# XiangFeng-Wen/STF-Unet

Hardware: AMD Instinct MI355X
Metric: training samples/sec (256x256 DCE-MRI frames) (higher is better)
Workload: dtype bf16; 1 GPU; cfg2 UNet(in=8,base_c=64) 256x256 train step; model=UNet, global_batch=64, per_gpu_batch=64, seq_len=8, parallelism=dp1, ddp_hook=False

## Files before the change

include/stfunet.h:

```cpp
#ifndef STFUNET_H
#define STFUNET_H
#include <stddef.h>
#include <stdint.h>

#ifdef __cplusplus
extern "C" {
#endif

typedef void* stf_stream_t;

typedef struct stf_conv_geom {
  int N;
  int Hs, Ws, Cs;
  int src_cstride;
  int Hd, Wd;
  int R, S;
  int stride, pad;
  int transposed;
} stf_conv_geom;

typedef struct stf_lstm_epi {
  const float* c_prev;
  float* c_out;
  void* h_out;
// ... 78 lines not shown
               int res_cstride, const float* res_scale, const float* res_shift, void* out,
               int out_cstride, void* pooled, stf_stream_t stream);
int stf_bn_bwd_tiles(int N, int H, int W, int C, int groups, int pooled);
int stf_bn_bwd_reduce(const void* dz, int dz_cstride, const void* dpool, const void* y,
                      int y_cstride, int N, int H, int W, int C, int groups,
                      const float* scale, const float* shift, const float* mean,
                      const float* invstd, int mask_mode, const void* mask_src,
                      int mask_cstride, void* g_out, float* partial, stf_stream_t stream);
int stf_bn_bwd_finalize(float* partial, int tiles, int groups, int C, int64_t M,
                        const float* gamma, const float* mean, const float* invstd,
                        float* dgamma, float* dbeta, float* coef, stf_stream_t stream);
typedef struct stf_bn_gsum_desc {
  const float* partial;
  float* dgamma;
  float* dbeta;
  int tiles, groups, C;
} stf_bn_gsum_desc;
int stf_bn_groupsum_batch(const stf_bn_gsum_desc* descs, int count, stf_stream_t stream);
int stf_bn_bwd_apply_tiles(int64_t M, int C);
int stf_bn_bwd_apply(const void* g, int g_cstride, const void* y, int y_cstride, int64_t M,
                     int C, int groups, const float* mask_scale, const float* mask_shift,
                     const float* coef, void* dy, int dy_cstride, float* bias_partial,
                     float* dbias, stf_stream_t stream);

int stf_head_fwd(const void* y, int N, int H, int W, int C, const float* scale,
                 const float* shift, const float* w, const float* bias, int classes,
                 float* logits, stf_stream_t stream);
int stf_head_bwd(const float* dlogits, const void* y, int N, int H, int W, int C,
                 const float* scale, const float* shift, const float* mean,
                 const float* invstd, const float* w, int classes, void* g_out,
                 float* bn_partial, float* head_partial, float* dw, float* db,
                 stf_stream_t stream);
int stf_head_tiles(int N, int H, int W, int C);

int stf_loss_scratch_floats(int N, int classes);
int stf_loss_fwd(const float* logits, const int64_t* target, int N, int H, int W,
                 int classes, float* terms, float* loss, stf_stream_t stream);
int stf_loss_bwd(const float* logits, const int64_t* target, int N, int H, int W,
                 int classes, const float* terms, const float* grad_out, float* dlogits,
                 stf_stream_t stream);
int stf_loss_opt_scratch_floats(int N, int classes);
int stf_loss_opt_fwd(const float* logits, const int64_t* target, int N, int H, int W, int classes,
                     const float* class_weight, int ignore_index, int dice, float* terms,
                     float* loss, stf_stream_t stream);
int stf_loss_opt_bwd(const float* logits, const int64_t* target, int N, int H, int W, int classes,
                     const float* class_weight, int ignore_index, int dice, const float* terms,
                     const float* grad_out, float* dlogits, stf_stream_t stream);
int stf_head_mc_fwd(const void* y, int N, int H, int W, int C, const float* scale,
                    const float* shift, const float* w, const float* bias, int classes,
                    float* logits, stf_stream_t stream);
int stf_head_mc_bwd(const float* dlogits, const void* y, int N, int H, int W, int C,
                    const float* scale, const float* shift, const float* mean,
                    const float* invstd, const float* w, int classes, void* g_out,
                    float* bn_partial, float* head_partial, float* dw, float* db,
                    stf_stream_t stream);
int stf_loss_mc_scratch_floats(int N, int classes);
int stf_loss_mc_fwd(const float* logits, const int64_t* target, int N, int H, int W, int classes,
                    const float* class_weight, int ignore_index, int dice, float* terms,
                    float* loss, stf_stream_t stream);
int stf_loss_mc_bwd(const float* logits, const int64_t* target, int N, int H, int W, int classes,
                    const float* class_weight, int ignore_index, int dice, const float* terms,
                    const float* grad_out, float* dlogits, stf_stream_t stream);
int stf_loss_ft_scratch_floats(int N, int classes);
int stf_loss_ft_fwd(const float* logits, const int64_t* target, int N, int H, int W, int classes,
                    const float* class_weight, int ignore_index, int dice, float focal_gamma,
                    float tversky_alpha, float tversky_beta, float* terms, float* loss,
// ... 185 lines not shown
```

stf-unet_amd/csrc/bn.hip:

```cpp
#include <algorithm>

#include "common.h"
#include "../../include/stfunet.h"
#include "reduce.h"

namespace {

constexpr int NT = 256;

STF_DEV void bn_fin_store(int g, int c, int C, double mu, double var, const float* gamma, const float* beta,
                          float eps, float* mean, float* invstd, float* scale, float* shift) {
  const float inv = (float)(1.0 / sqrt(var + (double)eps));
  const float sc = gamma[c] * inv;
  mean[g * C + c] = (float)mu;
  invstd[g * C + c] = inv;
  scale[g * C + c] = sc;
  shift[g * C + c] = beta[c] - (float)mu * sc;
}

STF_DEV void bn_fin_fwd_out(float* base, int g, int c, int G, int C, long Mg, double s1, double s2,
                            const float* gamma, const float* beta, float mom, float eps, float* rm, float* rv,
                            float* mean, float* invstd, float* scale, float* shift) {
  const double mu = s1 / Mg;
  double var = s2 / Mg - mu * mu;
  if (var < 0) var = 0;
  bn_fin_store(g, c, C, mu, var, gamma, beta, eps, mean, invstd, scale, shift);
  if (G == 1) {
    if (!rm) return;
    const double unb = Mg > 1 ? var * Mg / (Mg - 1) : var;
    rm[c] = (1.f - mom) * rm[c] + mom * (float)mu;
    rv[c] = (1.f - mom) * rv[c] + mom * (float)unb;
  } else {
    base[c] = (float)mu;
    base[C + c] = (float)var;
  }
}

// ... 11 lines not shown
    stf::fold16_pair(base, S, 2L * C, C, c, cok, red, s1, s2);
    if (lead)
      bn_fin_fwd_out(base, g, c, G, C, Mg, s1, s2, gamma, beta, mom, eps, rm, rv, mean, invstd, scale, shift);
    return;
  }
  if (!lead) return;
  bn_fin_store(g, c, C, rm ? rm[c] : 0.f, rv ? rv[c] : 1.f, gamma, beta, eps, mean, invstd, scale, shift);
}

STF_DEV void bn_fin_bwd_out(float* base, int g, int c, int G, int C, long Mg, double s1, double s2,
                            const float* gamma, const float* mean, const float* invstd, float* dgamma, float* dbeta,
                            float* coef) {
  const double is = invstd[g * C + c];
  const double A = (double)gamma[c] * is;
  const double B = -A * is * s2 / Mg;
  const double Cc = -A * s1 / Mg + A * is * mean[g * C + c] * s2 / Mg;
  coef[(size_t)g * 3 * C + c] = (float)A;
  coef[(size_t)g * 3 * C + C + c] = (float)B;
  coef[(size_t)g * 3 * C + 2 * C + c] = (float)Cc;
  if (G == 1) {
    if (dgamma) dgamma[c] = (float)s2;
    if (dbeta) dbeta[c] = (float)s1;
  } else {
    base[c] = (float)s1;
    base[C + c] = (float)s2;
  }
}


STF_DEV void load_pair(const float* a, const float* b, int g, int C, int cg, float (&va)[8], float (&vb)[8]) {
  load8f(a + (size_t)g * C, cg * 8, va);
  load8f(b + (size_t)g * C, cg * 8, vb);
}
STF_DEV void load_coef(const float* coef, int g, int C, int cg, float (&A)[8], float (&B)[8], float (&Cc)[8]) {
  load8f(coef + (size_t)g * 3 * C, cg * 8, A);
  load8f(coef + (size_t)g * 3 * C + C, cg * 8, B);
  load8f(coef + (size_t)g * 3 * C + 2 * C, cg * 8, Cc);
}

STF_DEV void bn_affine8(float (&v)[8], const float (&sc)[8], const float (&sh)[8], int relu, int res_mode,
                        const uint4* rq, const float (&rs)[8], const float (&rh)[8]) {
#pragma unroll
  for (int j = 0; j < 8; ++j) v[j] = v[j] * sc[j] + sh[j];
  if (res_mode) {
    float r[8];
    unpack8(*rq, r);
    if (res_mode == 2) {
#pragma unroll
      for (int j = 0; j < 8; ++j) r[j] = r[j] * rs[j] + rh[j];
    }
#pragma unroll
    for (int j = 0; j < 8; ++j) v[j] += r[j];
  }
  if (relu) {
#pragma unroll
    for (int j = 0; j < 8; ++j) v[j] = fmaxf(v[j], 0.f);
  }
}

STF_DEV void bn_acc8(int mask, float (&d)[8], const float (&y)[8], const float (&sc)[8], const float (&sh)[8],
                     const float* mk, const float (&mu)[8], const float (&is)[8], float (&sg)[8], float (&sgx)[8]) {
#pragma unroll
  for (int j = 0; j < 8; ++j) {
    bool keep = true;
    if (mask == 1) keep = y[j] * sc[j] + sh[j] > 0.f;
    else if (mask == 2) keep = mk[j] > 0.f;
    const float gj = keep ? d[j] : 0.f;
    d[j] = gj;
    sg[j] += gj;
    sgx[j] += gj * (y[j] - mu[j]) * is[j];
  }
}

STF_DEV void bn_dy8(bool mask, float (&gv)[8], const float (&y)[8], const float (&ms)[8], const float (&mh)[8],
                    const float (&A)[8], const float (&B)[8], const float (&Cc)[8], float (&sb)[8]) {
#pragma unroll
  for (int j = 0; j < 8; ++j) {
    const float gj = (mask && !(y[j] * ms[j] + mh[j] > 0.f)) ? 0.f : gv[j];
    gv[j] = A[j] * gj + B[j] * y[j] + Cc[j];
    sb[j] += gv[j];
  }
}

template <int Q = 1, int NTH, int RW>
STF_DEV void bn_block_fold(float (&red)[NTH][RW], const float (&s0)[8], const float (&s1)[8], int C, int stride,
                           int gy, float* __restrict__ out) {
  constexpr int H = (RW - 1) / 8;
#pragma unroll
  for (int j = 0; j < 8; ++j) {
    red[threadIdx.x][j] = s0[j];
    if (H == 2) red[threadIdx.x][8 + j] = s1[j];
  }
  __syncthreads();
  const size_t row = (size_t)gy * gridDim.x + blockIdx.x;
  for (int c = threadIdx.x; c < C; c += NTH) {
    const int gg = c >> 3, j = c & 7;
    float a = 0.f, b = 0.f;
    for (int t = Q * gg; t < NTH; t += stride)
      for (int q = 0; q < Q; ++q) {
        a += red[t + q][j];
        if (H == 2) b += red[t + q][8 + j];
      }
    out[row * H * C + c] = a;
    if (H == 2) out[row * H * C + C + c] = b;
  }
}

template <bool POOL>
__global__ void bn_act_kernel(const uint16_t* __restrict__ y, int ycs, long N, int H, int W, int C, long Mg,
                              const float* scale, const float* shift, int relu, int res_mode,
                              const uint16_t* __restrict__ res, int rcs, const float* __restrict__ rscale,
                              const float* __restrict__ rshift, uint16_t* __restrict__ out, int ocs,
                              uint16_t* __restrict__ pooled) {
// ... 841 lines not shown
```

stf-unet_amd/csrc/head.hip:

```cpp
#include "common.h"
#include "../../include/stfunet.h"
#include "reduce.h"

namespace {

constexpr int NT = 256;

STF_DEV float lane_group_sum(float v, int CG) {
  if (CG >= 2) v += dpp_f<0xB1>(v);
  if (CG >= 4) v += dpp_f<0x4E>(v);
  if (CG >= 8) v += dpp_f<0x141>(v);
  if (CG >= 16) v += dpp_f<0x140>(v);
  for (int o = 16; o < CG; o <<= 1) v += __shfl_xor(v, o, 64);
  return v;
}

int head_tiles(long units) {
  long t = (units + NT - 1) / NT;
  return (int)(t < 1 ? 1 : (t > 1024 ? 1024 : t));
}

template <int K>
__global__ void head_fwd_kernel(const uint16_t* __restrict__ y, long P, int HW, int C,
                                const float* __restrict__ scale, const float* __restrict__ shift,
                                const float* __restrict__ w, const float* __restrict__ bias,
                                float* __restrict__ logits) {
  constexpr int U = 4;
  const int CG = C / 8, cgs = __builtin_ctz(CG);
  const int units = (int)(P * CG);
  const int cg = (int)((blockIdx.x * NT + threadIdx.x) & (CG - 1));
  float sc[8], sh[8], wk[K][8], bk[K];
  load8f(scale, cg * 8, sc);
  load8f(shift, cg * 8, sh);
#pragma unroll
  for (int k = 0; k < K; ++k) { load8f(w + k * C, cg * 8, wk[k]); bk[k] = bias[k]; }
  const int stride = gridDim.x * NT;
  for (int u0 = blockIdx.x * NT; u0 < units; u0 += stride * U) {
    uint4 raw[U];
#pragma unroll
    for (int r = 0; r < U; ++r) {
      const int u = u0 + r * stride + threadIdx.x;
      raw[r] = u < units ? *reinterpret_cast<const uint4*>(y + (size_t)(u >> cgs) * C + cg * 8) : make_uint4(0, 0, 0, 0);
    }
#pragma unroll
    for (int r = 0; r < U; ++r) {
      const int u = u0 + r * stride + threadIdx.x;
      float v[8], acc[K];
      unpack8(raw[r], v);
#pragma unroll
      for (int k = 0; k < K; ++k) acc[k] = 0.f;
#pragma unroll
      for (int j = 0; j < 8; ++j) {
        const float a = fmaxf(v[j] * sc[j] + sh[j], 0.f);
#pragma unroll
        for (int k = 0; k < K; ++k) acc[k] += a * wk[k][j];
      }
#pragma unroll
      for (int k = 0; k < K; ++k) acc[k] = lane_group_sum(acc[k], CG);
      if (u < units && cg == 0) {
        const int pix = u >> cgs, n = pix / HW, hw = pix - n * HW;
#pragma unroll
        for (int k = 0; k < K; ++k) logits[(size_t)(n * K + k) * HW + hw] = acc[k] + bk[k];
      }
    }
  }
}

template <int K>
__global__ void head_bwd_kernel(const float* __restrict__ dlogits, const uint16_t* __restrict__ y, long P, int HW,
                                int C, const float* __restrict__ scale, const float* __restrict__ shift,
                                const float* __restrict__ mean, const float* __restrict__ invstd,
                                const float* __restrict__ w, uint16_t* __restrict__ g_out,
                                float* __restrict__ bn_partial, float* __restrict__ head_partial) {
  constexpr int NV = 16 + 8 * K + K;
  __shared__ float red[NT][NV + 1];
  const int CG = C / 8, cgs = __builtin_ctz(CG);
  const int units = (int)(P * CG);
  const int gt = blockIdx.x * NT + threadIdx.x;
  const int cg = gt & (CG - 1);
  float sc[8], sh[8], mu[8], is[8], wk[K][8];
  load8f(scale, cg * 8, sc);
  load8f(shift, cg * 8, sh);
  load8f(mean, cg * 8, mu);
  load8f(invstd, cg * 8, is);
#pragma unroll
  for (int k = 0; k < K; ++k) load8f(w + k * C, cg * 8, wk[k]);
  float sg[8] = {0, 0, 0, 0, 0, 0, 0, 0}, sgx[8] = {0, 0, 0, 0, 0, 0, 0, 0}, dw[K][8], db[K];
#pragma unroll
  for (int k = 0; k < K; ++k) {
    db[k] = 0.f;
#pragma unroll
    for (int j = 0; j < 8; ++j) dw[k][j] = 0.f;
  }
  constexpr int U = 1;
  const int S = gridDim.x * NT;
  for (int u0 = gt; u0 < units; u0 += S * U) {
    float dlr[U][K];
    uint4 yr[U];
    int pixr[U];
#pragma unroll
    for (int r = 0; r < U; ++r) {
      const int u = u0 + r * S;
      const bool ok = u < units;
      const int pix = ok ? u >> cgs : 0, n = pix / HW, hw = pix - n * HW;
      pixr[r] = ok ? pix : -1;
#pragma unroll
      for (int k = 0; k < K; ++k) dlr[r][k] = ok ? dlogits[(size_t)(n * K + k) * HW + hw] : 0.f;
      yr[r] = ok ? *reinterpret_cast<const uint4*>(y + (size_t)pix * C + cg * 8) : make_uint4(0, 0, 0, 0);
    }
#pragma unroll
    for (int r = 0; r < U; ++r) {
    if (pixr[r] < 0) continue;
    const int pix = pixr[r];
    const float* dl = dlr[r];
    float v[8], g[8];
    unpack8(yr[r], v);
#pragma unroll
    for (int j = 0; j < 8; ++j) {
      const float z = v[j] * sc[j] + sh[j];
      const float a = fmaxf(z, 0.f);
      float da = 0.f;
#pragma unroll
      for (int k = 0; k < K; ++k) { da += dl[k] * wk[k][j]; dw[k][j] += dl[k] * a; }
      g[j] = z > 0.f ? da : 0.f;
      sg[j] += g[j];
      sgx[j] += g[j] * (v[j] - mu[j]) * is[j];
    }
    if (cg == 0) {
#pragma unroll
      for (int k = 0; k < K; ++k) db[k] += dl[k];
    }
    *reinterpret_cast<uint4*>(g_out + (size_t)pix * C + cg * 8) = pack8(g);
    }
  }
#pragma unroll
  for (int j = 0; j < 8; ++j) { red[threadIdx.x][j] = sg[j]; red[threadIdx.x][8 + j] = sgx[j]; }
#pragma unroll
  for (int k = 0; k < K; ++k) {
#pragma unroll
    for (int j = 0; j < 8; ++j) red[threadIdx.x][16 + k * 8 + j] = dw[k][j];
    red[threadIdx.x][16 + 8 * K + k] = db[k];
  }
  __syncthreads();
  for (int c = threadIdx.x; c < C; c += NT) {
    const int gg = c / 8, j = c - gg * 8;
    float a = 0.f, b = 0.f;
    for (int t = gg; t < NT; t += CG) { a += red[t][j]; b += red[t][8 + j]; }
    bn_partial[(size_t)blockIdx.x * 2 * C + c] = a;
    bn_partial[(size_t)blockIdx.x * 2 * C + C + c] = b;
  }
  const int HC = K * (C + 1);
  for (int e = threadIdx.x; e < HC; e += NT) {
    float a = 0.f;
    if (e < K * C) {
      const int k = e / C, c = e - k * C, gg = c / 8, j = c - gg * 8;
      for (int t = gg; t < NT; t += CG) a += red[t][16 + k * 8 + j];
    } else {
      const int k = e - K * C;
      for (int t = 0; t < NT; t += CG) a += red[t][16 + 8 * K + k];
    }
    head_partial[(size_t)blockIdx.x * HC + e] = a;
  }
}

__global__ void sum_tiles_kernel(const float* __restrict__ partial, int tiles, int C, int split,
// ... 84 lines not shown
                                                         float* __restrict__ bn_partial,
                                                         float* __restrict__ head_partial) {
  extern __shared__ __attribute__((aligned(16))) float sm[];
  const int CG = C / 8, cgs = __builtin_ctz(CG);
  const int units = (int)(P * CG);
  const int gt = blockIdx.x * NT + threadIdx.x;
  const int cg = gt & (CG - 1);
  const int K4 = (K + 3) & ~3;
  for (int i = threadIdx.x; i < K4 * C; i += NT) sm[i] = i < K * C ? w[i] : 0.f;
  float sc[8], sh[8], mu[8], is[8];
  load8f(scale, cg * 8, sc);
  load8f(shift, cg * 8, sh);
  load8f(mean, cg * 8, mu);
  load8f(invstd, cg * 8, is);
  float sg[8] = {0, 0, 0, 0, 0, 0, 0, 0}, sgx[8] = {0, 0, 0, 0, 0, 0, 0, 0}, dw[KP][8], db[KP];
#pragma unroll
  for (int k = 0; k < KP; ++k) {
    db[k] = 0.f;
#pragma unroll
    for (int j = 0; j < 8; ++j) dw[k][j] = 0.f;
  }
  __syncthreads();
  const float* wc = sm + cg * 8;
  const int S = gridDim.x * NT;
  for (int u = gt; u < units; u += S) {
    const int pix = u >> cgs, n = pix / HW, hw = pix - n * HW;
    const float* dp = dlogits + (size_t)n * K * HW + hw;
    float dl[KP];
#pragma unroll
    for (int k = 0; k < KP; ++k) dl[k] = k < K ? dp[(size_t)k * HW] : 0.f;
    const uint4 yr = *reinterpret_cast<const uint4*>(y + (size_t)pix * C + cg * 8);
    float v[8], a[8], g[8];
    unpack8(yr, v);
#pragma unroll
    for (int j = 0; j < 8; ++j) {
      a[j] = v[j] * sc[j] + sh[j];
      g[j] = 0.f;
    }
#pragma unroll
    for (int kb = 0; kb < KP; kb += 4) {
      if (kb < K) {
#pragma unroll
        for (int k = kb; k < kb + 4; ++k) {
          float wk[8];
          load8f(wc, k * C, wk);
#pragma unroll
          for (int j = 0; j < 8; ++j) {
            g[j] += dl[k] * wk[j];
            dw[k][j] += dl[k] * fmaxf(a[j], 0.f);
          }
        }
      }
    }
#pragma unroll
    for (int j = 0; j < 8; ++j) {
      g[j] = a[j] > 0.f ? g[j] : 0.f;
      sg[j] += g[j];
      sgx[j] += g[j] * (v[j] - mu[j]) * is[j];
    }
    if (cg == 0) {
#pragma unroll
      for (int k = 0; k < KP; ++k) db[k] += dl[k];
    }
    *reinterpret_cast<uint4*>(g_out + (size_t)pix * C + cg * 8) = pack8(g);
  }
  float(*red)[MCRED] = reinterpret_cast<float(*)[MCRED]>(sm);
  const int HC = K * (C + 1);
  __syncthreads();
#pragma unroll
  for (int j = 0; j < 8; ++j) { red[threadIdx.x][j] = sg[j]; red[threadIdx.x][8 + j] = sgx[j]; }
#pragma unroll
  for (int k = 0; k < KP; ++k) red[threadIdx.x][16 + k] = db[k];
  __syncthreads();
  for (int c = threadIdx.x; c < C; c += NT) {
    const int gg = c / 8, j = c - gg * 8;
    float a = 0.f, b = 0.f;
    for (int t = gg; t < NT; t += CG) { a += red[t][j]; b += red[t][8 + j]; }
    bn_partial[(size_t)blockIdx.x * 2 * C + c] = a;
    bn_partial[(size_t)blockIdx.x * 2 * C + C + c] = b;
  }
  if ((int)threadIdx.x < K) {
    float a = 0.f;
    for (int t = 0; t < NT; t += CG) a += red[t][16 + threadIdx.x];
    head_partial[(size_t)blockIdx.x * HC + K * C + threadIdx.x] = a;
  }
#pragma unroll
  for (int kb = 0; kb < KP; kb += 4) {
    if (kb < K) {
      __syncthreads();
#pragma unroll
      for (int kk = 0; kk < 4; ++kk)
#pragma unroll
        for (int j = 0; j < 8; ++j) red[threadIdx.x][kk * 8 + j] = dw[kb + kk][j];
      __syncthreads();
      for (int e = threadIdx.x; e < 4 * C; e += NT) {
        const int kk = e / C, c = e - kk * C, gg = c / 8, j = c - gg * 8;
        if (kb + kk < K) {
          float a = 0.f;
          for (int t = gg; t < NT; t += CG) a += red[t][kk * 8 + j];
          head_partial[(size_t)blockIdx.x * HC + (size_t)(kb + kk) * C + c] = a;
        }
      }
    }
  }
}

bool mc_classes_ok(int classes) { return classes >= 1 && classes <= MCK; }

constexpr long MCBLOCKS = 4096;
bool head_mc_units_ok(long HW, long units) { return HW < (1L << 31) && units < (1L << 31) - 2 * MCBLOCKS * NT; }

size_t head_mc_lds_bytes(int C, int classes, bool bwd) {
  size_t f = (size_t)((classes + 3) & ~3) * C;
  if (bwd && f < (size_t)NT * MCRED) f = (size_t)NT * MCRED;
  return f * sizeof(float);
}

}

extern "C" int stf_head_tiles(int N, int H, int W, int C) { return head_tiles((long)N * H * W * (C / 8)); }

extern "C" int stf_head_fwd(const void* y, int N, int H, int W, int C, const float* scale, const float* shift,
                            const float* w, const float* bias, int classes, float* logits, stf_stream_t stream) {
  if (!head_ok(C)) return STF_EINVAL;
  const long P = (long)N * H * W, units = P * (C / 8);
  if (units >= (1L << 31)) return STF_EINVAL;
  long blocks = (units + NT - 1) / NT;
  if (blocks > 8192) blocks = 8192;
  hipStream_t s = (hipStream_t)stream;
  STF_KDISPATCH(classes, hipLaunchKernelGGL(head_fwd_kernel<KK>, dim3(blocks), dim3(NT), 0, s, (const uint16_t*)y,
                                            P, H * W, C, scale, shift, w, bias, logits));
  STF_CHECK_LAUNCH();
  return 0;
}

// ... 8 lines not shown
  STF_KDISPATCH(classes, hipLaunchKernelGGL(head_bwd_kernel<KK>, dim3(tiles), dim3(NT), 0, s, dlogits,
                                            (const uint16_t*)y, P, H * W, C, scale, shift, mean, invstd, w,
                                            (uint16_t*)g_out, bn_partial, head_partial));
  STF_CHECK_LAUNCH();
  const int HC = classes * (C + 1);
  const int S = stf::colsum_stage1(head_partial, tiles, HC, s);
  hipLaunchKernelGGL(sum_tiles_kernel, dim3((HC + 255) / 256), dim3(256), 0, s, head_partial, S, HC, classes * C,
                     dw, db);
  STF_CHECK_LAUNCH();
  return 0;
}

extern "C" int stf_head_mc_fwd(const void* y, int N, int H, int W, int C, const float* scale, const float* shift,
                               const float* w, const float* bias, int classes, float* logits, stf_stream_t stream) {
  if (C < 8 || !head_ok(C) || !mc_classes_ok(classes) || N < 1 || H < 1 || W < 1) return STF_EINVAL;
  if (!y || !scale || !shift || !w || !bias || !logits) return STF_EINVAL;
  const long P = (long)N * H * W, units = P * (C / 8);
  if (!head_mc_units_ok((long)H * W, units)) return STF_EINVAL;
  long blocks = (units + NT - 1) / NT;
  if (blocks > MCBLOCKS) blocks = MCBLOCKS;
  hipStream_t s = (hipStream_t)stream;
  STF_KPDISPATCH(classes, hipLaunchKernelGGL(head_mc_fwd_kernel<KP>, dim3(blocks), dim3(NT),
                                             head_mc_lds_bytes(C, classes, false), s, (const uint16_t*)y, P, H * W, C,
                                             classes, scale, shift, w, bias, logits));
  STF_CHECK_LAUNCH();
  return 0;
}

extern "C" int stf_head_mc_bwd(const float* dlogits, const void* y, int N, int H, int W, int C, const float* scale,
                               const float* shift, const float* mean, const float* invstd, const float* w,
                               int classes, void* g_out, float* bn_partial, float* head_partial, float* dw, float* db,
                               stf_stream_t stream) {
  if (C < 8 || !head_ok(C) || !mc_classes_ok(classes) || N < 1 || H < 1 || W < 1) return STF_EINVAL;
  if (!dlogits || !y || !scale || !shift || !mean || !invstd || !w || !g_out || !bn_partial || !head_partial || !dw ||
      !db)
    return STF_EINVAL;
  if (!head_mc_units_ok((long)H * W, (long)N * H * W * (C / 8))) return STF_EINVAL;
  const long P = (long)N * H * W;
  const int tiles = stf_head_tiles(N, H, W, C);
  hipStream_t s = (hipStream_t)stream;
  STF_KPDISPATCH(classes, hipLaunchKernelGGL(head_mc_bwd_kernel<KP>, dim3(tiles), dim3(NT),
                                             head_mc_lds_bytes(C, classes, true), s, dlogits, (const uint16_t*)y, P,
                                             H * W, C, classes, scale, shift, mean, invstd, w, (uint16_t*)g_out,
                                             bn_partial, head_partial));
  STF_CHECK_LAUNCH();
  const int HC = classes * (C + 1);
  const int S = stf::colsum_stage1(head_partial, tiles, HC, s);
  hipLaunchKernelGGL(sum_tiles_kernel, dim3((HC + 255) / 256), dim3(256), 0, s, head_partial, S, HC, classes * C,
                     dw, db);
  STF_CHECK_LAUNCH();
  return 0;
}
```

stf-unet_amd/stfunet/_lib.py:

```python
import contextlib
import ctypes
import os

import torch

_HERE = os.path.dirname(os.path.abspath(__file__))
LIB_PATH = os.path.join(_HERE, "libstfunet_hip.so")
LIB_PATH = os.environ.get("STF_LIB", LIB_PATH)
LIB_PATH_F16 = os.environ.get("STF_LIB_F16", os.path.join(os.path.dirname(LIB_PATH), "libstfunet_hip_f16.so"))
LIB_PATHS = {torch.bfloat16: LIB_PATH, torch.float16: LIB_PATH_F16}
STORAGE_CODE = {torch.bfloat16: 0, torch.float16: 1}

BUILD_INFO = os.path.join(_HERE, "build_info.json")
_SRC_DIRS = (os.path.join(_HERE, "..", "csrc"), os.path.join(_HERE, "..", "..", "include"))


def _sha(paths):
    import hashlib
    h = hashlib.sha256()
    for p in paths:
        h.update(os.path.basename(p).encode())
        with open(p, "rb") as f:
            h.update(f.read())
    return h.hexdigest()[:16]
# ... 59 lines not shown
    _fields_ = [("g", ConvGeom), ("dy", P), ("dy_cstride", c_int), ("Nout", c_int), ("x", P),
                ("ws", P), ("splits", c_int), ("grid_blocks", c_int)]


class Seg(ctypes.Structure):
    _fields_ = [("off", c_int64), ("len", c_int64)]


_SIGS = {
    "stf_igemm_stat_tiles": (c_int, [ctypes.POINTER(IgemmArgs)]),
    "stf_igemm_ws_bytes": (c_size_t, [ctypes.POINTER(IgemmArgs)]),
    "stf_igemm_bnr_tiles": (c_int, [ctypes.POINTER(IgemmArgs)]),
    "stf_igemm_kernel_name": (ctypes.c_char_p, [ctypes.POINTER(IgemmArgs)]),
    "stf_wgrad_kernel_name": (ctypes.c_char_p, [ctypes.POINTER(WgradArgs)]),
    "stf_igemm": (c_int, [ctypes.POINTER(IgemmArgs), P]),
    "stf_wgrad_plan": (c_int, [ctypes.POINTER(WgradArgs), ctypes.POINTER(c_int), ctypes.POINTER(c_size_t)]),
    "stf_wgrad": (c_int, [ctypes.POINTER(WgradArgs), P]),
    "stf_wgrad_reduce": (c_int, [P, c_int, c_int, c_int, c_int, c_int, P, P]),
    "stf_channel_sum": (c_int, [P, c_int, c_int, c_int, P, P, P]),
    "stf_bn_finalize": (c_int, [P, c_int, c_int, c_int, c_int64, P, P, c_float, c_float, P, P, P, P, P, P, P]),
    "stf_bn_running_batch": (c_int, [P, c_int, P]),
    "stf_bn_groupsum_batch": (c_int, [P, c_int, P]),
    "stf_bn_act": (c_int, [P, c_int, c_int, c_int, c_int, c_int, c_int, P, P, c_int, P, c_int, P, P, P, c_int, P,
                           P]),
    "stf_bn_bwd_tiles": (c_int, [c_int, c_int, c_int, c_int, c_int, c_int]),
    "stf_bn_bwd_reduce": (c_int, [P, c_int, P, P, c_int, c_int, c_int, c_int, c_int, c_int, P, P, P, P, c_int, P,
                                  c_int, P, P, P]),
    "stf_bn_bwd_finalize": (c_int, [P, c_int, c_int, c_int, c_int64, P, P, P, P, P, P, P]),
    "stf_bn_bwd_apply_tiles": (c_int, [c_int64, c_int]),
    "stf_bn_bwd_apply": (c_int, [P, c_int, P, c_int, c_int64, c_int, c_int, P, P, P, P, c_int, P, P, P]),
    "stf_head_fwd": (c_int, [P, c_int, c_int, c_int, c_int, P, P, P, P, c_int, P, P]),
    "stf_head_bwd": (c_int, [P, P, c_int, c_int, c_int, c_int, P, P, P, P, P, c_int, P, P, P, P, P, P]),
    "stf_head_tiles": (c_int, [c_int, c_int, c_int, c_int]),
    "stf_loss_scratch_floats": (c_int, [c_int, c_int]),
    "stf_loss_fwd": (c_int, [P, P, c_int, c_int, c_int, c_int, P, P, P]),
    "stf_loss_bwd": (c_int, [P, P, c_int, c_int, c_int, c_int, P, P, P, P]),
    "stf_loss_opt_scratch_floats": (c_int, [c_int, c_int]),
    "stf_loss_opt_fwd": (c_int, [P, P, c_int, c_int, c_int, c_int, P, c_int, c_int, P, P, P]),
    "stf_loss_opt_bwd": (c_int, [P, P, c_int, c_int, c_int, c_int, P, c_int, c_int, P, P, P, P]),
    "stf_head_mc_fwd": (c_int, [P, c_int, c_int, c_int, c_int, P, P, P, P, c_int, P, P]),
    "stf_head_mc_bwd": (c_int, [P, P, c_int, c_int, c_int, c_int, P, P, P, P, P, c_int, P, P, P, P, P, P]),
    "stf_loss_mc_scratch_floats": (c_int, [c_int, c_int]),
    "stf_loss_mc_fwd": (c_int, [P, P, c_int, c_int, c_int, c_int, P, c_int, c_int, P, P, P]),
    "stf_loss_mc_bwd": (c_int, [P, P, c_int, c_int, c_int, c_int, P, c_int, c_int, P, P, P, P]),
    "stf_loss_ft_scratch_floats": (c_int, [c_int, c_int]),
    "stf_loss_ft_fwd": (c_int, [P, P, c_int, c_int, c_int, c_int, P, c_int, c_int, c_float, c_float, c_float, P, P,
                                P]),
    "stf_loss_ft_bwd": (c_int, [P, P, c_int, c_int, c_int, c_int, P, c_int, c_int, c_float, c_float, c_float, P, P,
                                P, P]),
    "stf_adamw": (c_int, [P, P, P, P, c_int64, c_float, c_float, c_float, c_float, c_float, c_float, c_float,
                          P]),
    "stf_adamw_dev": (c_int, [P, P, P, P, c_int64, P, c_float, c_float, c_float, c_float, P]),
    "stf_adamw_amp": (c_int, [P, P, P, P, c_int64, P, P, P, c_float, c_float, c_float, c_float, P]),
    "stf_grad_norm_rows": (c_int, [c_int64]),
    "stf_grad_norm": (c_int, [P, P, P, c_int, P, c_float, P, P, P]),
    "stf_grad_scale": (c_int, [P, P, P, c_int, P, P]),
    "stf_adamw_clip": (c_int, [P, P, P, P, c_int64, P, P, P, P, c_float, c_float, c_float, c_float, P]),
    "stf_pack_input": (c_int, [P, c_int, c_int, c_int, c_int, c_int, P, P]),
    "stf_pack_weight": (c_int, [P, c_int, c_int, c_int, c_int, c_int, c_int, P, P]),
    "stf_pack_weights": (c_int, [P, c_int, c_int64, P]),
    "stf_augment_frames": (c_int, [P, P, c_int, P, P, c_int, c_int, c_float, c_float, P, P]),
    "stf_augment_masks": (c_int, [P, P, c_int, P, c_int, P, P]),
    "stf_pack_tiles": (c_int, [c_int, c_int, c_int, c_int, c_int, c_int]),
    "stf_pack_weights_tiled": (c_int, [P, c_int, c_int, P]),
    "stf_pack_sequence": (c_int, [P, c_int, c_int, c_int, c_int, c_int, c_int, c_int, c_int, P, P]),
    "stf_eval_counts": (c_int, [P, P, c_int, c_int, c_int64, c_int64, P, P, P]),
# ... 149 lines not shown
```

stf-unet_amd/stfunet/nhwc.py:

```python
import contextlib
import ctypes
import os
from dataclasses import dataclass

import torch

from . import _lib
from ._lib import BnrEpi, ConvGeom, IgemmArgs, WgradArgs, call, stream

BF16 = torch.bfloat16


def sdt():
    return _lib.storage_dtype()


def _p(t):
    return t.data_ptr() if t is not None else None


class KernelTimer:

    def __init__(self, only=None, log=False):
        self.rec = {}
# ... 645 lines not shown
    if out is not None:
        out.check()
        assert (out.N, out.H, out.W, out.C) == (y.N, y.H, y.W, C)
    if mask_relu:
        assert out is not None
    call("stf_bn_bwd_apply", g.ptr(), g.cs, y.ptr(), y.cs, y.M, C, G, _p(st.scale) if mask_relu else None,
         _p(st.shift) if mask_relu else None, _p(coef), dst.ptr(), dst.cs, _p(bpart), _p(dbias), stream())
    return dst


MAX_CLASSES = 16


def check_num_classes(K):
    if not 1 <= K <= MAX_CLASSES:
        raise ValueError(f"num_classes={K}: the head and criterion kernels take 1 to {MAX_CLASSES} classes")


def _head_entry(name, K):
    check_num_classes(K)
    return f"stf_head_mc_{name}" if K > 4 else f"stf_head_{name}"


def head_fwd(y: Feat, st: BNState, conv, logits):
    y.check()
    K = conv.out_channels
    assert y.cs == y.C and y.off == 0 and tuple(logits.shape) == (y.N, K, y.H, y.W)
    head_w = conv.weight.detach().reshape(K, -1).contiguous()
    call(_head_entry("fwd", K), y.ptr(), y.N, y.H, y.W, y.C, _p(st.scale), _p(st.shift), _p(head_w), _p(conv.bias.detach()),
         K, _p(logits), stream())
    return head_w


def head_bwd(dlogits, y: Feat, st: BNState, head_w, dweight, dbias):
    y.check()
    K, C, dev = dlogits.shape[1], y.C, dlogits.device
    assert dlogits.dtype == torch.float32 and dlogits.is_contiguous() and tuple(dlogits.shape) == (y.N, K, y.H, y.W)
    tiles = _lib.load().stf_head_tiles(y.N, y.H, y.W, C)
    g = new_feat(y.N, y.H, y.W, C, dev)
    bnp = empty(tiles * 2 * C, torch.float32, dev)
    hp = empty((tiles + 1) * K * (C + 1), torch.float32, dev)
    call(_head_entry("bwd", K), _p(dlogits), y.ptr(), y.N, y.H, y.W, C, _p(st.scale), _p(st.shift), _p(st.mean),
         _p(st.invstd), _p(head_w), K, g.ptr(), _p(bnp), _p(hp), _p(dweight), _p(dbias), stream())
    return g, bnp, tiles
```

stf-unet_amd/stfunet/unet.py:

```python

import torch
import torch.nn as nn

from . import nhwc
from .nhwc import Feat, new_feat
from .program import Program, Saved as _Saved, conv_bn, conv_pair_backward, run_step


def _double_conv(cin, cout):
    return nn.Sequential(nn.Conv2d(cin, cout, 3, padding=1), nn.BatchNorm2d(cout), nn.ReLU(inplace=True),
                         nn.Conv2d(cout, cout, 3, padding=1), nn.BatchNorm2d(cout), nn.ReLU(inplace=True))


def _cpad(c):
    return (c + 7) // 8 * 8


class DoubleConvProgram:

    def __init__(self, blk, name=""):
        self.blk = blk
        self.cout = blk[0].out_channels
        self.name = name

# ... 93 lines not shown
        for i, (up, dec) in enumerate(zip(self.ups, self.decs)):
            cat = S.cats[3 - i]
            Clo = dec.cout
            wt = nhwc.pack_weight(up.weight, 2)
            nhwc.igemm(cur, wt, 4 * Clo, cat.slice(0, Clo), 1, 1, 1, 0, bias=up.bias.detach(), scatter2x2=True)
            S.dec_in.append(cur if fm[f"up{4 - i}"].need_w else None)
            last = i == 3
            if not last:
                out = new_feat(cat.N, cat.H, cat.W, Clo, dev)
                S.dec.append(dec.forward(cat, training, need_bwd and fm.runs(dec.name), out=out))
                cur = out
            else:
                s = dec.forward(cat, training, True)
                if not fm.runs(dec.name):
                    s.src = s.y1 = s.a1 = None
                S.dec.append(s)
        s = S.dec[-1]
        K = m.out_conv.out_channels
        logits = nhwc.empty((N, K, H, W), torch.float32, dev)
        S.head_w = nhwc.head_fwd(s.y2, s.bn2, m.out_conv, logits)
        S.cats = None
        if not need_bwd:
            S.enc = S.dec = None
        nhwc.flush_batches_tracked()
        return logits, (S if need_bwd else None)

    def _backward(self, S, dlogits):
        m = self.m
        gv = self.flat.grad_view
        dev = dlogits.device
        dlogits = dlogits.contiguous().float()
        fm = S.fmap
        s = S.dec[-1]
        g, bnp, tiles = nhwc.head_bwd(dlogits, s.y2, s.bn2, S.head_w, gv(m.out_conv.weight), gv(m.out_conv.bias))
        dec1 = self.decs[3]
        dcats = [None] * 4
        if fm.runs("dec1"):
            dy2 = nhwc.bn_backward_from_partial(g, s.y2, s.bn2, dec1.blk[4], bnp, tiles, gv(dec1.blk[4].weight),
                                                gv(dec1.blk[4].bias), gv(dec1.blk[3].bias))
            dcats[0] = dec1.backward(s, self.flat, fm["dec1"].need_din, dy2=dy2, dsrc_stats=True,
                                     need_w=fm["dec1"].need_w)
        self._done(dec1.blk)
        for i in (3, 2, 1, 0):
            up, nu = self.ups[i], fm[f"up{4 - i}"]
            dsrc = None
            if dcats[3 - i] is not None:
                dcat, cst, ctiles = dcats[3 - i]
                dcats[3 - i] = dcat
                Clo = self.decs[i].cout
                dup = dcat.slice(0, Clo)
                if nu.need_w:
                    nhwc.wgrad(S.dec_in[i], dup, 2, 2, 2, 0, gv(up.weight))
                    nhwc.stat_sums(cst, ctiles, dcat.C, 0, Clo, gv(up.bias))
                if nu.need_din:
                    dsrc = new_feat(dcat.N, dcat.H // 2, dcat.W // 2, up.in_channels, dev)
                    nhwc.igemm(dup, nhwc.pack_weight(up.weight, 3), dsrc.C, dsrc, 2, 2, 2, 0)
            self._done(up)
            if i > 0:
                dec = self.decs[i - 1]
                if fm.runs(dec.name):
                    dcats[4 - i] = dec.backward(S.dec[i - 1], self.flat, fm[dec.name].need_din, dz=dsrc,
                                                dsrc_stats=True, need_w=fm[dec.name].need_w)
                self._done(dec.blk)
            else:
                d_b = dsrc
        dpool = None
        if fm.runs("bottleneck"):
            dpool = self.bott.backward(S.bott, self.flat, fm["bottleneck"].need_din, dz=d_b,
                                       need_w=fm["bottleneck"].need_w)
        self._done(self.bott.blk)
        for j in (3, 2, 1, 0):
            lvl = self.levels[j]
# ... 45 lines not shown
```

Baseline: 2725 samples/s.

## Recompute head gradient inside BN backward apply instead of storing it

In the training path, the head backward kernel can now skip writing the full-resolution bf16 gradient tensor. A new fused kernel, head_bn_apply, recomputes that gradient from dlogits, the head weights and the saved activation, then applies the BN backward coefficients to produce dy directly. The aim is to remove a large write and re-read of a 64-channel 256x256 feature map per step. The cost is a second pass over dlogits and repeated head math. The new path no longer passes the preceding conv bias gradient, and it uses a slot-dependent FMA pattern meant to reproduce the old rounding.

```diff
diff --git a/include/stfunet.h b/include/stfunet.h
--- a/include/stfunet.h
+++ b/include/stfunet.h
@@ -134,6 +134,9 @@
                  float* bn_partial, float* head_partial, float* dw, float* db,
                  stf_stream_t stream);
 int stf_head_tiles(int N, int H, int W, int C);
+int stf_head_bn_apply(const float* dlogits, const void* y, int N, int H, int W, int C,
+                      const float* scale, const float* shift, const float* w, int classes,
+                      const float* coef, void* dy, stf_stream_t stream);
 
 int stf_loss_scratch_floats(int N, int classes);
 int stf_loss_fwd(const float* logits, const int64_t* target, int N, int H, int W,
diff --git a/stf-unet_amd/csrc/bn.hip b/stf-unet_amd/csrc/bn.hip
--- a/stf-unet_amd/csrc/bn.hip
+++ b/stf-unet_amd/csrc/bn.hip
@@ -3,6 +3,7 @@
 #include "common.h"
 #include "../../include/stfunet.h"
 #include "reduce.h"
+#include "bn_dy.h"
 
 namespace {
 
@@ -80,11 +81,6 @@
   load8f(a + (size_t)g * C, cg * 8, va);
   load8f(b + (size_t)g * C, cg * 8, vb);
 }
-STF_DEV void load_coef(const float* coef, int g, int C, int cg, float (&A)[8], float (&B)[8], float (&Cc)[8]) {
-  load8f(coef + (size_t)g * 3 * C, cg * 8, A);
-  load8f(coef + (size_t)g * 3 * C + C, cg * 8, B);
-  load8f(coef + (size_t)g * 3 * C + 2 * C, cg * 8, Cc);
-}
 
 STF_DEV void bn_affine8(float (&v)[8], const float (&sc)[8], const float (&sh)[8], int relu, int res_mode,
                         const uint4* rq, const float (&rs)[8], const float (&rh)[8]) {
@@ -117,16 +113,6 @@
     d[j] = gj;
     sg[j] += gj;
     sgx[j] += gj * (y[j] - mu[j]) * is[j];
-  }
-}
-
-STF_DEV void bn_dy8(bool mask, float (&gv)[8], const float (&y)[8], const float (&ms)[8], const float (&mh)[8],
-                    const float (&A)[8], const float (&B)[8], const float (&Cc)[8], float (&sb)[8]) {
-#pragma unroll
-  for (int j = 0; j < 8; ++j) {
-    const float gj = (mask && !(y[j] * ms[j] + mh[j] > 0.f)) ? 0.f : gv[j];
-    gv[j] = A[j] * gj + B[j] * y[j] + Cc[j];
-    sb[j] += gv[j];
   }
 }
 
diff --git a/stf-unet_amd/csrc/bn_dy.h b/stf-unet_amd/csrc/bn_dy.h
--- /dev/null
+++ b/stf-unet_amd/csrc/bn_dy.h
@@ -0,0 +1,30 @@
+#pragma once
+#include "common.h"
+
+STF_DEV void load_coef(const float* coef, int g, int C, int cg, float (&A)[8], float (&B)[8], float (&Cc)[8]) {
+  load8f(coef + (size_t)g * 3 * C, cg * 8, A);
+  load8f(coef + (size_t)g * 3 * C + C, cg * 8, B);
+  load8f(coef + (size_t)g * 3 * C + 2 * C, cg * 8, Cc);
+}
+
+STF_DEV void bn_dy8(bool mask, float (&gv)[8], const float (&y)[8], const float (&ms)[8], const float (&mh)[8],
+                    const float (&A)[8], const float (&B)[8], const float (&Cc)[8], float (&sb)[8]) {
+#pragma unroll
+  for (int j = 0; j < 8; ++j) {
+    const float gj = (mask && !(y[j] * ms[j] + mh[j] > 0.f)) ? 0.f : gv[j];
+    gv[j] = A[j] * gj + B[j] * y[j] + Cc[j];
+    sb[j] += gv[j];
+  }
+}
+
+STF_DEV void bn_dy8_as_apply(int slot, float (&gv)[8], const float (&y)[8], const float (&A)[8],
+                             const float (&B)[8], const float (&Cc)[8]) {
+#pragma clang fp contract(off)
+#pragma unroll
+  for (int j = 0; j < 8; ++j) {
+    const bool fused = j < 5 || (j == 5 && slot != 3) || (j == 6 && slot == 3);
+    const float by = B[j] * y[j];
+    const float t = fused ? __builtin_fmaf(A[j], gv[j], by) : A[j] * gv[j] + by;
+    gv[j] = t + Cc[j];
+  }
+}
diff --git a/stf-unet_amd/csrc/head.hip b/stf-unet_amd/csrc/head.hip
--- a/stf-unet_amd/csrc/head.hip
+++ b/stf-unet_amd/csrc/head.hip
@@ -1,6 +1,7 @@
 #include "common.h"
 #include "../../include/stfunet.h"
 #include "reduce.h"
+#include "bn_dy.h"
 
 namespace {
 
@@ -64,6 +65,27 @@
       }
     }
   }
+}
+
+template <int KN, class WRow>
+STF_DEV void head_g8(const float (&v)[8], const float (&sc)[8], const float (&sh)[8], const float (&dl)[KN], int K,
+                     WRow wrow, float (&z)[8], float (&g)[8]) {
+#pragma unroll
+  for (int j = 0; j < 8; ++j) {
+    z[j] = __builtin_fmaf(v[j], sc[j], sh[j]);
+    g[j] = 0.f;
+  }
+#pragma unroll
+  for (int k = 0; k < KN; ++k) {
+    if ((k & ~3) < K) {
+      float wk[8];
+      wrow(k, wk);
+#pragma unroll
+      for (int j = 0; j < 8; ++j) g[j] = __builtin_fmaf(dl[k], wk[j], g[j]);
+    }
+  }
+#pragma unroll
+  for (int j = 0; j < 8; ++j) g[j] = z[j] > 0.f ? g[j] : 0.f;
 }
 
 template <int K>
@@ -113,16 +135,17 @@
     if (pixr[r] < 0) continue;
     const int pix = pixr[r];
     const float* dl = dlr[r];
-    float v[8], g[8];
+    float v[8], z[8], g[8];
     unpack8(yr[r], v);
+    head_g8<K>(v, sc, sh, dlr[r], K, [&](int k, float (&o)[8]) {
+#pragma unroll
+      for (int j = 0; j < 8; ++j) o[j] = wk[k][j];
+    }, z, g);
 #pragma unroll
     for (int j = 0; j < 8; ++j) {
-      const float z = v[j] * sc[j] + sh[j];
-      const float a = fmaxf(z, 0.f);
-      float da = 0.f;
-#pragma unroll
-      for (int k = 0; k < K; ++k) { da += dl[k] * wk[k][j]; dw[k][j] += dl[k] * a; }
-      g[j] = z > 0.f ? da : 0.f;
+      const float a = fmaxf(z[j], 0.f);
+#pragma unroll
+      for (int k = 0; k < K; ++k) dw[k][j] += dl[k] * a;
       sg[j] += g[j];
       sgx[j] += g[j] * (v[j] - mu[j]) * is[j];
     }
@@ -130,7 +153,7 @@
 #pragma unroll
       for (int k = 0; k < K; ++k) db[k] += dl[k];
     }
-    *reinterpret_cast<uint4*>(g_out + (size_t)pix * C + cg * 8) = pack8(g);
+    if (g_out) *reinterpret_cast<uint4*>(g_out + (size_t)pix * C + cg * 8) = pack8(g);
     }
   }
 #pragma unroll
@@ -281,29 +304,18 @@
     const uint4 yr = *reinterpret_cast<const uint4*>(y + (size_t)pix * C + cg * 8);
     float v[8], a[8], g[8];
     unpack8(yr, v);
-#pragma unroll
-    for (int j = 0; j < 8; ++j) {
-      a[j] = v[j] * sc[j] + sh[j];
-      g[j] = 0.f;
-    }
+    head_g8<KP>(v, sc, sh, dl, K, [&](int k, float (&o)[8]) { load8f(wc, k * C, o); }, a, g);
 #pragma unroll
     for (int kb = 0; kb < KP; kb += 4) {
       if (kb < K) {
 #pragma unroll
-        for (int k = kb; k < kb + 4; ++k) {
-          float wk[8];
-          load8f(wc, k * C, wk);
-#pragma unroll
-          for (int j = 0; j < 8; ++j) {
-            g[j] += dl[k] * wk[j];
-            dw[k][j] += dl[k] * fmaxf(a[j], 0.f);
-          }
-        }
+        for (int k = kb; k < kb + 4; ++k)
+#pragma unroll
+          for (int j = 0; j < 8; ++j) dw[k][j] += dl[k] * fmaxf(a[j], 0.f);
       }
     }
 #pragma unroll
     for (int j = 0; j < 8; ++j) {
-      g[j] = a[j] > 0.f ? g[j] : 0.f;
       sg[j] += g[j];
       sgx[j] += g[j] * (v[j] - mu[j]) * is[j];
     }
@@ -311,7 +323,7 @@
 #pragma unroll
       for (int k = 0; k < KP; ++k) db[k] += dl[k];
     }
-    *reinterpret_cast<uint4*>(g_out + (size_t)pix * C + cg * 8) = pack8(g);
+    if (g_out) *reinterpret_cast<uint4*>(g_out + (size_t)pix * C + cg * 8) = pack8(g);
   }
   float(*red)[MCRED] = reinterpret_cast<float(*)[MCRED]>(sm);
   const int HC = K * (C + 1);
@@ -350,6 +362,72 @@
           head_partial[(size_t)blockIdx.x * HC + (size_t)(kb + kk) * C + c] = a;
         }
       }
+    }
+  }
+}
+
+template <int KN, bool LDSW>
+__global__ __launch_bounds__(NT) void head_bn_apply_kernel(const float* __restrict__ dlogits,
+                                                           const uint16_t* __restrict__ y, long P, int HW, int C,
+                                                           int K, const float* __restrict__ scale,
+                                                           const float* __restrict__ shift,
+                                                           const float* __restrict__ w,
+                                                           const float* __restrict__ coef,
+                                                           uint16_t* __restrict__ dy) {
+  extern __shared__ __attribute__((aligned(16))) float wl[];
+  constexpr int U = 2;
+  constexpr int KR = LDSW ? 1 : KN;
+  const int CG = C / 8, cgs = __builtin_ctz(CG);
+  const int Kc = LDSW ? K : KN;
+  const long units = P * CG;
+  const int cg = (int)threadIdx.x & (CG - 1);
+  float sc[8], sh[8], A[8], B[8], Cc[8], wk[KR][8];
+  load8f(scale, cg * 8, sc);
+  load8f(shift, cg * 8, sh);
+  load_coef(coef, 0, C, cg, A, B, Cc);
+  if constexpr (LDSW) {
+    const int K4 = (Kc + 3) & ~3;
+    for (int i = threadIdx.x; i < K4 * C; i += NT) wl[i] = i < Kc * C ? w[i] : 0.f;
+    __syncthreads();
+  } else {
+#pragma unroll
+    for (int k = 0; k < KR; ++k) load8f(w + k * C, cg * 8, wk[k]);
+  }
+  const float* wc = wl + cg * 8;
+  const long S = (long)gridDim.x * NT * U;
+  for (long u0 = (long)blockIdx.x * NT * U + threadIdx.x; u0 < units; u0 += S) {
+    float dl[U][KN];
+    uint4 yq[U];
+#pragma unroll
+    for (int r = 0; r < U; ++r) {
+      const long u = u0 + r * NT;
+      const bool ok = u < units;
+      const int pix = ok ? (int)(u >> cgs) : 0, n = pix / HW, hw = pix - n * HW;
+      const float* dp = dlogits + (size_t)n * Kc * HW + hw;
+#pragma unroll
+      for (int k = 0; k < KN; ++k) dl[r][k] = ok && k < Kc ? dp[(size_t)k * HW] : 0.f;
+      yq[r] = ok ? *reinterpret_cast<const uint4*>(y + (size_t)pix * C + cg * 8) : make_uint4(0, 0, 0, 0);
+    }
+#pragma unroll
+    for (int r = 0; r < U; ++r) {
+      const long u = u0 + r * NT;
+      if (u >= units) break;
+      float v[8], z[8], g[8];
+      unpack8(yq[r], v);
+      head_g8<KN>(v, sc, sh, dl[r], Kc, [&](int k, float (&o)[8]) {
+        if constexpr (LDSW) {
+          load8f(wc, k * C, o);
+        } else {
+#pragma unroll
+          for (int j = 0; j < 8; ++j) o[j] = wk[k][j];
+        }
+      }, z, g);
+#pragma unroll
+      for (int j = 0; j < 8; ++j) asm volatile("" : "+v"(g[j]));
+      const uint4 gq = pack8(g);
+      unpack8(gq, g);
+      bn_dy8_as_apply((int)(u >> 8) & 3, g, v, A, B, Cc);
+      *reinterpret_cast<uint4*>(dy + (size_t)(u >> cgs) * C + cg * 8) = pack8(g);
     }
   }
 }
@@ -424,8 +502,7 @@
                                int classes, void* g_out, float* bn_partial, float* head_partial, float* dw, float* db,
                                stf_stream_t stream) {
   if (C < 8 || !head_ok(C) || !mc_classes_ok(classes) || N < 1 || H < 1 || W < 1) return STF_EINVAL;
-  if (!dlogits || !y || !scale || !shift || !mean || !invstd || !w || !g_out || !bn_partial || !head_partial || !dw ||
-      !db)
+  if (!dlogits || !y || !scale || !shift || !mean || !invstd || !w || !bn_partial || !head_partial || !dw || !db)
     return STF_EINVAL;
   if (!head_mc_units_ok((long)H * W, (long)N * H * W * (C / 8))) return STF_EINVAL;
   const long P = (long)N * H * W;
@@ -443,3 +520,26 @@
   STF_CHECK_LAUNCH();
   return 0;
 }
+
+extern "C" int stf_head_bn_apply(const float* dlogits, const void* y, int N, int H, int W, int C, const float* scale,
+                                 const float* shift, const float* w, int classes, const float* coef, void* dy,
+                                 stf_stream_t stream) {
+  if (C < 8 || !head_ok(C) || !mc_classes_ok(classes) || N < 1 || H < 1 || W < 1) return STF_EINVAL;
+  if (!dlogits || !y || !scale || !shift || !w || !coef || !dy) return STF_EINVAL;
+  const long P = (long)N * H * W, units = P * (C / 8);
+  if (classes <= 4 ? units >= (1L << 31) : !head_mc_units_ok((long)H * W, units)) return STF_EINVAL;
+  long blocks = (units + 2 * NT - 1) / (2 * NT);
+  if (blocks > 8192) blocks = 8192;
+  hipStream_t s = (hipStream_t)stream;
+  if (classes <= 4) {
+    STF_KDISPATCH(classes, hipLaunchKernelGGL((head_bn_apply_kernel<KK, false>), dim3(blocks), dim3(NT), 0, s, dlogits,
+                                              (const uint16_t*)y, P, H * W, C, classes, scale, shift, w, coef,
+                                              (uint16_t*)dy));
+  } else {
+    STF_KPDISPATCH(classes, hipLaunchKernelGGL((head_bn_apply_kernel<KP, true>), dim3(blocks), dim3(NT),
+                                               head_mc_lds_bytes(C, classes, false), s, dlogits, (const uint16_t*)y,
+                                               P, H * W, C, classes, scale, shift, w, coef, (uint16_t*)dy));
+  }
+  STF_CHECK_LAUNCH();
+  return 0;
+}
diff --git a/stf-unet_amd/stfunet/_lib.py b/stf-unet_amd/stfunet/_lib.py
--- a/stf-unet_amd/stfunet/_lib.py
+++ b/stf-unet_amd/stfunet/_lib.py
@@ -115,6 +115,7 @@
     "stf_head_fwd": (c_int, [P, c_int, c_int, c_int, c_int, P, P, P, P, c_int, P, P]),
     "stf_head_bwd": (c_int, [P, P, c_int, c_int, c_int, c_int, P, P, P, P, P, c_int, P, P, P, P, P, P]),
     "stf_head_tiles": (c_int, [c_int, c_int, c_int, c_int]),
+    "stf_head_bn_apply": (c_int, [P, P, c_int, c_int, c_int, c_int, P, P, P, c_int, P, P, P]),
     "stf_loss_scratch_floats": (c_int, [c_int, c_int]),
     "stf_loss_fwd": (c_int, [P, P, c_int, c_int, c_int, c_int, P, P, P]),
     "stf_loss_bwd": (c_int, [P, P, c_int, c_int, c_int, c_int, P, P, P, P]),
diff --git a/stf-unet_amd/stfunet/nhwc.py b/stf-unet_amd/stfunet/nhwc.py
--- a/stf-unet_amd/stfunet/nhwc.py
+++ b/stf-unet_amd/stfunet/nhwc.py
@@ -701,14 +701,34 @@
     return head_w
 
 
-def head_bwd(dlogits, y: Feat, st: BNState, head_w, dweight, dbias):
+def head_bwd(dlogits, y: Feat, st: BNState, head_w, dweight, dbias, store_g=True):
     y.check()
     K, C, dev = dlogits.shape[1], y.C, dlogits.device
     assert dlogits.dtype == torch.float32 and dlogits.is_contiguous() and tuple(dlogits.shape) == (y.N, K, y.H, y.W)
     tiles = _lib.load().stf_head_tiles(y.N, y.H, y.W, C)
-    g = new_feat(y.N, y.H, y.W, C, dev)
+    g = new_feat(y.N, y.H, y.W, C, dev) if store_g else None
     bnp = empty(tiles * 2 * C, torch.float32, dev)
     hp = empty((tiles + 1) * K * (C + 1), torch.float32, dev)
     call(_head_entry("bwd", K), _p(dlogits), y.ptr(), y.N, y.H, y.W, C, _p(st.scale), _p(st.shift), _p(st.mean),
-         _p(st.invstd), _p(head_w), K, g.ptr(), _p(bnp), _p(hp), _p(dweight), _p(dbias), stream())
+         _p(st.invstd), _p(head_w), K, g.ptr() if store_g else None, _p(bnp), _p(hp), _p(dweight), _p(dbias),
+         stream())
     return g, bnp, tiles
+
+
+HEAD_RECOMPUTE_MIN_BYTES = 32 << 20
+
+
+def head_recompute_pays(y: Feat):
+    return 2 * y.M * y.C >= HEAD_RECOMPUTE_MIN_BYTES
+
+
+def bn_backward_head(dlogits, y: Feat, st: BNState, head_w, bn, part, tiles, dgamma, dbeta):
+    y.check()
+    K, C = dlogits.shape[1], y.C
+    check_num_classes(K)
+    assert st.training and st.groups == 1 and y.cs == C and y.off == 0
+    coef = _bn_bwd_coef(y, st, bn, part, tiles, dgamma, dbeta)
+    dy = new_feat(y.N, y.H, y.W, C, y.buf.device)
+    call("stf_head_bn_apply", _p(dlogits), y.ptr(), y.N, y.H, y.W, C, _p(st.scale), _p(st.shift), _p(head_w), K,
+         _p(coef), dy.ptr(), stream())
+    return dy
diff --git a/stf-unet_amd/stfunet/unet.py b/stf-unet_amd/stfunet/unet.py
--- a/stf-unet_amd/stfunet/unet.py
+++ b/stf-unet_amd/stfunet/unet.py
@@ -149,12 +149,19 @@
         dlogits = dlogits.contiguous().float()
         fm = S.fmap
         s = S.dec[-1]
-        g, bnp, tiles = nhwc.head_bwd(dlogits, s.y2, s.bn2, S.head_w, gv(m.out_conv.weight), gv(m.out_conv.bias))
         dec1 = self.decs[3]
+        store_g = fm.runs("dec1") and not (s.bn2.training and nhwc.head_recompute_pays(s.y2))
+        g, bnp, tiles = nhwc.head_bwd(dlogits, s.y2, s.bn2, S.head_w, gv(m.out_conv.weight), gv(m.out_conv.bias),
+                                      store_g=store_g)
         dcats = [None] * 4
         if fm.runs("dec1"):
-            dy2 = nhwc.bn_backward_from_partial(g, s.y2, s.bn2, dec1.blk[4], bnp, tiles, gv(dec1.blk[4].weight),
-                                                gv(dec1.blk[4].bias), gv(dec1.blk[3].bias))
+            bn2 = dec1.blk[4]
+            if store_g:
+                dy2 = nhwc.bn_backward_from_partial(g, s.y2, s.bn2, bn2, bnp, tiles, gv(bn2.weight), gv(bn2.bias),
+                                                    gv(dec1.blk[3].bias))
+            else:
+                dy2 = nhwc.bn_backward_head(dlogits, s.y2, s.bn2, S.head_w, bn2, bnp, tiles, gv(bn2.weight),
+                                            gv(bn2.bias))
             dcats[0] = dec1.backward(s, self.flat, fm["dec1"].need_din, dy2=dy2, dsrc_stats=True,
                                      need_w=fm["dec1"].need_w)
         self._done(dec1.blk)
```

After: 2744 samples/s, median of 6. About the same (+0.7%).
